# fbergama/wass

Hardware: AMD Instinct MI355X
Metric: stereo_pairs_per_sec (higher is better)
Workload: dtype u16

## Files before the change

### include/wass_gpu.h

```cpp
#ifndef WASS_GPU_H
#define WASS_GPU_H

#include <stddef.h>
#include <stdint.h>

#ifdef __cplusplus
extern "C" {
#endif

typedef enum {
    WASS_OK = 0,
    WASS_ERR_INVALID_ARG = -1,
    WASS_ERR_UNSUPPORTED = -2,
    WASS_ERR_NO_MEMORY = -3,
    WASS_ERR_DEVICE = -4,
    WASS_ERR_COST_OVERFLOW = -5,
    WASS_ERR_TOO_FEW_POINTS = -6
} wass_status;

typedef struct wass_ctx wass_ctx;

int wass_ctx_create(int device_id, wass_ctx** out);
int wass_device_count(int* n_devices);
void wass_ctx_destroy(wass_ctx* ctx);
// ... 123 lines not shown
typedef struct wass_debug_desc {
    int W0, H0;
    int roi_l[4], roi_r[4];
    const uint8_t* d_left_crop;
    const uint8_t* d_right_crop;
    const int16_t* d_disp16;
    const float* d_dispf;
    int num_disp, min_disp, disp_offset;
    double disparity_compensation;
    int quality;
} wass_debug_desc;
int wass_jpeg_encode_dev(wass_ctx* ctx, const uint8_t* d_pixels, int w, int h, int channels, size_t pitch_bytes, int quality,
                         uint8_t* h_dst, size_t capacity, size_t* nbytes);
int wass_debug_picture_size(const wass_debug_desc* desc, int k, int* width, int* height, int* channels);
int wass_debug_pictures_async(wass_ctx* ctx, const wass_mesh* mesh, const wass_debug_desc* desc, uint8_t* h_dst,
                              const size_t capacity[WASS_DEBUG_PICTURES], uint64_t* ticket);
int wass_debug_pictures_result(wass_ctx* ctx, uint64_t ticket, size_t nbytes[WASS_DEBUG_PICTURES]);

enum {
    WASS_CODE_NONE = 0,
    WASS_CODE_GREY = 1,
    WASS_CODE_OUTSIDE_IMAGE = 2,
    WASS_CODE_OUTSIDE_BBOX = 3,
    WASS_CODE_ANGLE = 4,
    WASS_CODE_TOO_CLOSE = 5,
    WASS_CODE_TOO_DISTANT = 6
};
int wass_mesh_reject_codes(wass_ctx* ctx, const wass_mesh* m, uint8_t* codes_out);
void wass_mesh_destroy(wass_mesh* m);
int wass_mesh_size(const wass_mesh* m, int* width, int* height);
int wass_mesh_download(wass_ctx* ctx, const wass_mesh* m, uint8_t* valid, double* p3d, uint8_t* gray);
int wass_mesh_upload(wass_ctx* ctx, int width, int height, const uint8_t* valid, const double* p3d,
                     const uint8_t* gray, wass_mesh** out);

int wass_mesh_zgap_percentile(wass_ctx* ctx, wass_mesh* m, double percentile, double* out, uint64_t* n_gaps);
int wass_mesh_keep_biggest_component(wass_ctx* ctx, wass_mesh* m, double zgap, uint64_t* size_out);
int wass_ransac_sample(int width, int height, int rounds, int32_t* uv_triplets);
int wass_ransac_sample_seeded(uint32_t seed, int width, int height, int rounds, int32_t* uv_triplets);
int wass_mesh_ransac_plane(wass_ctx* ctx, wass_mesh* m, const int32_t* uv_triplets, int rounds,
                           double thr, double plane_out[4], uint64_t* best_inliers, int* found);
int wass_mesh_crop_plane(wass_ctx* ctx, wass_mesh* m, const double plane[4], double thr, uint64_t* kept);
typedef struct {
    double xmin, xmax, ymin, ymax;
    double max_distance;
    int weight_by_distance;
    int central_third_only;
} wass_refine_params;
int wass_mesh_refine_plane(wass_ctx* ctx, wass_mesh* m, const wass_refine_params* rp,
                           double plane_out[4], uint64_t* n_inliers);
int wass_mesh_refinement_inliers(wass_ctx* ctx, wass_mesh* m, const wass_refine_params* rp, int every, double** xyz_out,
                                 uint64_t* n_out);
int wass_mesh_remove_outliers(wass_ctx* ctx, wass_mesh* m, double percentile, double* zgap_out, uint64_t* n_gaps,
                              uint64_t* size_out);
typedef struct {
    int      found;
    double   ransac_plane[4];
    uint64_t ransac_inliers;
    double   plane[4];
    uint64_t refine_inliers;
    uint64_t kept_after_ransac_crop, kept_final;
} wass_plane_result;
int wass_mesh_fit_plane(wass_ctx* ctx, wass_mesh* m, const int32_t* uv_triplets, int rounds, double ransac_thr,
                        const wass_refine_params* rp, double max_distance, wass_plane_result* out);
typedef struct {
    double   zgap;  uint64_t n_gaps, component_size;
    int      found, refine_ok;
    double   ransac_plane[4];  uint64_t ransac_inliers;
    double   plane[4];         uint64_t refine_inliers, kept_after_ransac_crop, kept_final;
    uint64_t n_points, xyzc_bytes;
    int      sgm_cost_overflow, sgm_timeout;
    uint64_t n_triangulated;
    uint64_t n_inliers_out;
    float stage_ms[5];
    int reserved;
    uint64_t inliers_text_bytes;
    uint32_t inliers_text_unsupported, reserved2;
} wass_frame_result;
int wass_mesh_finish_frame_async(wass_ctx* ctx, wass_mesh* m, double percentile, const int32_t* uv_triplets, int rounds,
                                 double ransac_thr, const wass_refine_params* rp, double max_distance, void* dst,
                                 size_t capacity);
int wass_mesh_finish_frame_async_ex(wass_ctx* ctx, wass_mesh* m, double percentile, const int32_t* uv_triplets, int rounds,
                                    double ransac_thr, const wass_refine_params* rp, double max_distance, void* dst,
                                    size_t capacity, double* inliers_dst, size_t inliers_capacity, int inliers_every,
                                    uint8_t* component_mask_dst);
int wass_mesh_finish_frame_async_ex2(wass_ctx* ctx, wass_mesh* m, double percentile, const int32_t* uv_triplets, int rounds,
                                     double ransac_thr, const wass_refine_params* rp, double max_distance, void* dst,
                                     size_t capacity, double* inliers_dst, size_t inliers_capacity, int inliers_every,
                                     uint8_t* component_mask_dst, char* inliers_text_dst, size_t inliers_text_capacity);
int wass_format_g6(double v, char* out);
int wass_ctx_frame_inliers(wass_ctx* ctx, double* dst, size_t capacity_points, uint64_t* n_out);
int wass_ctx_frame_result(wass_ctx* ctx, wass_frame_result* out);

void wass_RT_from_plane(const double plane[4], double R[9], double T[3], double Rinv[9], double Tinv[3]);
int wass_mesh_encode_xyzc(wass_ctx* ctx, wass_mesh* m, const double plane[4], void** bytes, size_t* nbytes);
int wass_mesh_encode_xyzc_to(wass_ctx* ctx, wass_mesh* m, const double plane[4], void* dst, size_t capacity,
                             size_t* nbytes);
int wass_mesh_encode_xyzc_async(wass_ctx* ctx, wass_mesh* m, const double plane[4], void* dst, size_t capacity,
                                size_t* nbytes);
void wass_free(void* p);

typedef struct {
    double R[9], T[3];
    double baseline;
    double xmin, xmax, ymin, ymax;
    int    width, height;
} wass_grid_setup;
// ... 210 lines not shown
```

### wass_amd/_lib.py

```python
from __future__ import annotations

import ctypes as C
import os

_HERE = os.path.dirname(os.path.abspath(__file__))
SO_PATH = os.environ.get("WASS_GPU_LIB") or os.path.join(_HERE, "libwassgpu.so")

WASS_OK = 0
WASS_ERR_COST_OVERFLOW = -5


class WassError(RuntimeError):
    def __init__(self, code: int, msg: str):
        super().__init__(f"libwassgpu error {code}: {msg}")
        self.code = code


class SgmParams(C.Structure):
    _fields_ = [(n, C.c_int) for n in (
        "min_disp", "num_disp", "win", "P1", "P2", "uniq_ratio", "disp12_max_diff", "prefilter_cap",
        "speckle_win", "speckle_range", "ndirs", "disp_offset")] + [("dense_scale", C.c_double)]


class SgmTimings(C.Structure):
# ... 69 lines not shown


def default_sgm_params(num_disp: int, ndirs: int = 5, min_disp: int = 1, win: int = 13, p1_mult: int = 2,
                       p2_mult: int = 64, disp_offset: int = 0) -> SgmParams:
    return SgmParams(min_disp, num_disp, win, p1_mult * win * win, p2_mult * win * win, 1, -1, 60, -70, 16,
                     ndirs, disp_offset, 1.0)


_vp, _i, _sz = C.c_void_p, C.c_int, C.c_size_t
SYMBOLS = {
    "wass_version": (C.c_char_p, []),
    "wass_ctx_create": (_i, [_i, C.POINTER(_vp)]),
    "wass_ctx_destroy": (None, [_vp]),
    "wass_last_error": (C.c_char_p, [_vp]),
    "wass_ctx_stream": (_vp, [_vp]),
    "wass_ctx_synchronize": (_i, [_vp]),
    "wass_ctx_set_debug": (_i, [_vp, _i]),
    "wass_ctx_set_tail_overlap": (_i, [_vp, _i]),
    "wass_sgm_disparity": (_i, [_vp, _vp, _vp, _i, _i, _sz, C.POINTER(SgmParams), _vp]),
    "wass_sgm_disparity_dev": (_i, [_vp, _vp, _vp, _i, _i, _sz, C.POINTER(SgmParams), _vp]),
    "wass_sgm_last_timings": (_i, [_vp, C.POINTER(SgmTimings)]),
    "wass_sgm_prev_timings": (_i, [_vp, C.POINTER(SgmTimings)]),
    "wass_sgm_call_count": (_i, [_vp, C.POINTER(C.c_uint64)]),
    "wass_sgm_call_timings": (_i, [_vp, C.c_uint64, C.POINTER(SgmTimings)]),
    "wass_sgm_debug_fetch": (_i, [_vp, _vp, _vp, _vp]),
    "wass_sgm_probe_vsum": (_i, [_vp, C.POINTER(C.c_float), C.POINTER(C.c_float)]),
    "wass_sgm_selftest": (_i, [_vp, _i, _i, _i, _i, C.POINTER(C.c_uint64)]),
    "wass_device_count": (_i, [C.POINTER(_i)]),
    "wass_ctx_set_kernel_events": (_i, [_vp, _i]),
    "wass_sgm_kernel_times": (_i, [_vp, C.c_char_p, C.c_size_t, C.POINTER(C.c_float), _i, C.POINTER(_i)]),
    "wass_disparity_postprocess": (_i, [_vp, _vp, _i, _i, C.POINTER(SgmParams), _i, _i, _i, _vp]),
    "wass_disparity_postprocess_dev": (_i, [_vp, _vp, _i, _i, C.POINTER(SgmParams), _i, _i, _i, _vp]),
    "wass_triangulate": (_i, [_vp, _vp, _i, _i, C.POINTER(_i), C.POINTER(_i), C.POINTER(Geom), _vp, _i, _i, _vp, _vp,
                              C.POINTER(TriParams), C.POINTER(_vp), C.POINTER(C.c_uint64)]),
    "wass_triangulate_dev": (_i, [_vp, _vp, _i, _i, C.POINTER(_i), C.POINTER(_i), C.POINTER(Geom), _vp, _i, _i, _vp, _vp,
                                  C.POINTER(TriParams), C.POINTER(_vp), C.POINTER(C.c_uint64)]),
    "wass_mesh_destroy": (None, [_vp]),
    "wass_mesh_size": (_i, [_vp, C.POINTER(_i), C.POINTER(_i)]),
    "wass_mesh_download": (_i, [_vp, _vp, _vp, _vp, _vp]),
    "wass_mesh_upload": (_i, [_vp, _i, _i, _vp, _vp, _vp, C.POINTER(_vp)]),
    "wass_mesh_zgap_percentile": (_i, [_vp, _vp, C.c_double, C.POINTER(C.c_double), C.POINTER(C.c_uint64)]),
    "wass_mesh_keep_biggest_component": (_i, [_vp, _vp, C.c_double, C.POINTER(C.c_uint64)]),
    "wass_ransac_sample": (_i, [_i, _i, _i, _vp]),
    "wass_ransac_sample_seeded": (_i, [C.c_uint32, _i, _i, _i, _vp]),
    "wass_mesh_ransac_plane": (_i, [_vp, _vp, _vp, _i, C.c_double, C.POINTER(C.c_double), C.POINTER(C.c_uint64),
                                    C.POINTER(_i)]),
    "wass_mesh_crop_plane": (_i, [_vp, _vp, C.POINTER(C.c_double), C.c_double, C.POINTER(C.c_uint64)]),
    "wass_large_gradient_mask": (_i, [_vp, _i, _i, _vp]),
    "wass_mesh_reject_codes": (_i, [_vp, _vp, _vp]),
    "wass_mesh_refine_plane": (_i, [_vp, _vp, C.POINTER(RefineParams), C.POINTER(C.c_double), C.POINTER(C.c_uint64)]),
    "wass_mesh_refinement_inliers": (_i, [_vp, _vp, C.POINTER(RefineParams), _i, C.POINTER(C.POINTER(C.c_double)), C.POINTER(C.c_uint64)]),
    "wass_mesh_remove_outliers": (_i, [_vp, _vp, C.c_double, C.POINTER(C.c_double), C.POINTER(C.c_uint64),
                                       C.POINTER(C.c_uint64)]),
    "wass_mesh_fit_plane": (_i, [_vp, _vp, _vp, _i, C.c_double, C.POINTER(RefineParams), C.c_double,
                                 C.POINTER(PlaneResult)]),
    "wass_RT_from_plane": (None, [C.POINTER(C.c_double)] * 5),
    "wass_mesh_encode_xyzc": (_i, [_vp, _vp, C.POINTER(C.c_double), C.POINTER(_vp), C.POINTER(_sz)]),
    "wass_mesh_encode_xyzc_to": (_i, [_vp, _vp, C.POINTER(C.c_double), _vp, _sz, C.POINTER(_sz)]),
    "wass_mesh_encode_xyzc_async": (_i, [_vp, _vp, C.POINTER(C.c_double), _vp, _sz, C.POINTER(_sz)]),
    "wass_mesh_finish_frame_async": (_i, [_vp, _vp, C.c_double, _vp, _i, C.c_double, C.POINTER(RefineParams), C.c_double, _vp, _sz]),
    "wass_mesh_finish_frame_async_ex": (_i, [_vp, _vp, C.c_double, _vp, _i, C.c_double, C.POINTER(RefineParams), C.c_double, _vp, _sz,
                                             _vp, _sz, _i, _vp]),
    "wass_mesh_finish_frame_async_ex2": (_i, [_vp, _vp, C.c_double, _vp, _i, C.c_double, C.POINTER(RefineParams), C.c_double, _vp, _sz,
                                              _vp, _sz, _i, _vp, _vp, _sz]),
    "wass_format_g6": (_i, [C.c_double, _vp]),
    "wass_ctx_frame_inliers": (_i, [_vp, _vp, _sz, C.POINTER(C.c_uint64)]),
    "wass_ctx_frame_result": (_i, [_vp, C.POINTER(FrameResult)]),
    "wass_device_alloc": (_i, [_vp, _sz, C.POINTER(_vp)]),
    "wass_device_free": (None, [_vp, _vp]),
    "wass_download": (_i, [_vp, _vp, _vp, _sz]),
    "wass_download_async": (_i, [_vp, _vp, _vp, _sz]),
    "wass_resize_cubic_u8_dev": (_i, [_vp, _vp, _i, _i, _sz, _vp, _i, _i]),
    "wass_jpeg_encode_dev": (_i, [_vp, _vp, _i, _i, _i, _sz, _i, _vp, _sz, C.POINTER(_sz)]),
    "wass_debug_pictures_async": (_i, [_vp, _vp, C.POINTER(DebugDesc), _vp, C.POINTER(_sz * 8), C.POINTER(C.c_uint64)]),
    "wass_debug_picture_size": (_i, [C.POINTER(DebugDesc), _i, C.POINTER(_i), C.POINTER(_i), C.POINTER(_i)]),
    "wass_debug_pictures_result": (_i, [_vp, C.c_uint64, C.POINTER(_sz * 8)]),
    "wass_pinned_alloc": (_i, [_vp, _sz, C.POINTER(_vp)]),
    "wass_pinned_free": (None, [_vp, _vp]),
    "wass_free": (None, [_vp]),
    "wass_mesh_grid_idw": (_i, [_vp, _vp, C.POINTER(GridSetup), _vp, _vp]),
    "wass_mesh_grid_idw_ex": (_i, [_vp, _vp, C.POINTER(GridSetup), _i, _vp, _vp]),
    "wass_dct_opts_default": (None, [C.POINTER(DctOpts)]),
    "wass_grid_dct": (_i, [_vp, _vp, _i, _i, C.POINTER(DctOpts), _vp, _vp, _vp, _vp, C.POINTER(DctInfo)]),
    "wass_grid_dct_dev": (_i, [_vp, _vp, _i, _i, C.POINTER(DctOpts), _vp, _vp, _vp, _vp, C.POINTER(DctInfo)]),
    "wass_mesh_grid_dct": (_i, [_vp, _vp, C.POINTER(GridSetup), _i, C.POINTER(DctOpts), _vp, _vp, _vp, _vp, _vp, C.POINTER(DctInfo)]),
    "wass_grid_dct_eval": (_i, [_vp, _vp, _i, _i, _i, C.c_double, _vp, _vp, C.POINTER(C.c_double), C.POINTER(C.c_double)]),
    "wass_grid_dct_batch": (_i, [_vp, _vp, _i, _i, _i, C.POINTER(DctOpts), _vp, _vp, _vp, _vp, C.POINTER(DctInfo), C.POINTER(_i)]),
    "wass_grid_dct_batch_dev": (_i, [_vp, _vp, _i, _i, _i, C.POINTER(DctOpts), _vp, _vp, _vp, _vp, C.POINTER(DctInfo), C.POINTER(_i)]),
    "wass_mesh_grid_cells_dev": (_i, [_vp, _vp, C.POINTER(GridSetup), _i, _vp]),
    "wass_grid_median_dev": (_i, [_vp, _vp, _vp, _i, _i, _i, _i, _vp]),
    "wass_grid_seq_create": (_i, [_vp, _i, _i, C.POINTER(_vp)]),
    "wass_grid_seq_push_dev": (_i, [_vp, _vp, _i, _vp]),
    "wass_grid_seq_finish": (_i, [_vp, _i, C.POINTER(GridSeqStats), _vp, _vp, _vp, _vp]),
    "wass_grid_seq_zero_mean_dev": (_i, [_vp, _vp, _i]),
    "wass_grid_seq_destroy": (None, [_vp]),
    "wass_spec3d_scratch_bytes": (_i, [_i, _i, _i, C.POINTER(_sz)]),
    "wass_spec3d_create": (_i, [_vp, _i, _i, _i, _vp, _vp, _vp, C.POINTER(_vp)]),
    "wass_spec3d_push": (_i, [_vp, _vp, _sz, _sz, C.c_double]),
    "wass_spec3d_push_dev": (_i, [_vp, _vp, _sz, _sz, C.c_double]),
    "wass_spec3d_finish": (_i, [_vp, C.c_double, _vp, C.POINTER(_i), C.POINTER(_i)]),
    "wass_spec3d_destroy": (None, [_vp]),
    "wass_spec1d_welch": (_i, [_vp, _vp, _i, _i, _i, C.c_double, C.c_double, _vp]),
    "wass_sosfiltfilt_scratch_bytes": (_i, [_i, _i, _i, _i, _i, _i, C.POINTER(_sz), C.POINTER(_i)]),
    "wass_sosfiltfilt": (_i, [_vp, _vp, _sz, _sz, _i, _i, _i, _vp, _i, _vp, _i, _i, _i, _vp, _sz, _sz]),
    "wass_sosfiltfilt_dev": (_i, [_vp, _vp, _sz, _sz, _i, _i, _i, _vp, _i, _vp, _i, _i, _i, _vp, _sz, _sz]),
    "wass_spatial_filter_scratch_bytes": (_i, [_i, _i, _i, C.POINTER(_sz)]),
# ... 91 lines not shown
```

### wass_amd/csrc/mesh.hip

```cpp
#include "common.h"
#include "fmt_g6.h"

#include <math.h>
#include <stdlib.h>
#include <mutex>
#include <new>
#include <vector>

namespace wass {

struct GeomDev {
    double Kl[9], Kr[9], R[9], T[3];
    int use_custom;
    double R1[9], R2[9], P1[12], P2[12], HLi[9], HRi[9];
    double comp_over_scale;
};

__device__ __forceinline__ void mulv(const double* M, const double* v, double* o)
{
    o[0] = M[0] * v[0] + M[1] * v[1] + M[2] * v[2];
    o[1] = M[3] * v[0] + M[4] * v[1] + M[5] * v[2];
    o[2] = M[6] * v[0] + M[7] * v[1] + M[8] * v[2];
}
__device__ __forceinline__ void tmulv(const double* M, const double* v, double* o)
// ... 274 lines not shown
            const unsigned int cm = (unsigned)((i % w) * h + (i / w));
            if (r == r0) { atomicAdd(&agg, (unsigned)len); atomicMin(&aggmin, cm); }
            else { atomicAdd(&size[r], (unsigned)len); atomicMin(&mincm[r], cm); }
        }
    }
    __syncthreads();
    if (threadIdx.x == 0 && agg) { atomicAdd(&size[r0], agg); atomicMin(&mincm[r0], aggmin); }
}
__global__ void __launch_bounds__(256) k_ccl_best(int n, const int* __restrict__ parent, const unsigned int* __restrict__ size,
                                                  const unsigned int* __restrict__ mincm, unsigned long long* __restrict__ best)
{
    const int i = blockIdx.x * 256 + threadIdx.x;
    unsigned long long key = 0;
    if (i < n && parent[i] == i) key = ((unsigned long long)size[i] << 32) | (unsigned long long)(0xFFFFFFFFu - mincm[i]);
    for (int o = 32; o > 0; o >>= 1) {
        const unsigned long long other = __shfl_down(key, o);
        key = other > key ? other : key;
    }
    if ((threadIdx.x & 63) == 0 && key) atomicMax(best, key);
}
__global__ void __launch_bounds__(256) k_ccl_keep(uint8_t* __restrict__ valid, int n, const int* __restrict__ parent,
                                                  const unsigned int* __restrict__ size, const unsigned int* __restrict__ mincm,
                                                  const unsigned long long* __restrict__ best)
{
    const int i = blockIdx.x * 256 + threadIdx.x;
    if (i >= n) return;
    const int r = parent[i];
    bool keep = false;
    if (r >= 0) {
        const unsigned long long key = ((unsigned long long)size[r] << 32) | (unsigned long long)(0xFFFFFFFFu - mincm[r]);
        keep = key == *best;
    }
    valid[i] = keep ? 1 : 0;
}

struct DevState {
    unsigned long long sel_k, sel_prefix, sel_total;
    int sel_hi_shift, sel_fail;
    double zgap;
    unsigned long long ccl_best;
    int ransac_found, pad0;
    unsigned long long ransac_best;
    double ransac_plane[4];
    double wsum, centroid[3], ninl;
    double plane[4];
    int refine_ok, pad1;
    double rtR[9], rtT[3], rtRinv[9], rtTinv[3];
    double mn[3], sc[3];
    unsigned int npts, have_plane;
    unsigned long long kept1, kept2;
    unsigned long long ntri;
    unsigned int ninl_sel, inl_text_bad;
    unsigned long long inl_text_bytes;
};

constexpr int GAP_HIST_COPIES = 4;
constexpr int GAP_BITS = 11, GAP_BINS = 1 << GAP_BITS, GAP_PASSES = 6;
__global__ void __launch_bounds__(256) k_gap_hist(const uint8_t* __restrict__ valid, const double* __restrict__ Z, int w, int h,
                                                  int shift, unsigned int mask, const DevState* __restrict__ ds,
                                                  unsigned int* __restrict__ hist)
{
    __shared__ unsigned int lh[GAP_BINS];
    for (int i = threadIdx.x; i < GAP_BINS; i += 256) lh[i] = 0;
    __syncthreads();
    const int hi_shift = ds->sel_hi_shift;
    const unsigned long long prefix = ds->sel_prefix;
    const int j = blockIdx.x * 256 + threadIdx.x;
    if (j >= 1 && j < w - 1)
        for (int i = 1 + blockIdx.y; i < h; i += gridDim.y) {
            const size_t c = (size_t)i * w + j, up = c - w;
            const uint8_t vc = valid[c], v0 = valid[up - 1], v1 = valid[up], v2 = valid[up + 1];
            const double z = Z[c], z0 = Z[up - 1], z1 = Z[up], z2 = Z[up + 1];
            if (!vc) continue;
            const double zn[3] = { z0, z1, z2 };
            const uint8_t vn[3] = { v0, v1, v2 };
#pragma unroll
            for (int k = 0; k < 3; ++k) {
                if (!vn[k]) continue;
                const unsigned long long key = (unsigned long long)__double_as_longlong(fabs(z - zn[k]));
                if (hi_shift < 64 && (key >> hi_shift) != prefix) continue;
                atomicAdd(&lh[(unsigned)(key >> shift) & mask], 1u);
            }
        }
    __syncthreads();
    unsigned int* mine = hist + (size_t)((blockIdx.x + blockIdx.y) % GAP_HIST_COPIES) * GAP_BINS;
    for (int i = threadIdx.x; i < GAP_BINS; i += 256)
        if (lh[i]) atomicAdd(&mine[i], lh[i]);
}
__global__ void __launch_bounds__(256) k_radix_pick(unsigned int* __restrict__ hist, int pass, int shift, int nbits,
                                                    double percentile, DevState* __restrict__ ds)
{
    __shared__ unsigned long long tot[256];
    const int nb = 1 << nbits, per = (nb + 255) / 256;
    for (int i = threadIdx.x; i < GAP_BINS; i += 256) {
        unsigned int t = hist[i];
        for (int cpy = 1; cpy < GAP_HIST_COPIES; ++cpy) t += hist[(size_t)cpy * GAP_BINS + i];
        hist[i] = t;
    }
    __syncthreads();
    unsigned long long s = 0;
    for (int b = threadIdx.x * per; b < min(nb, (threadIdx.x + 1) * per); ++b) s += hist[b];
    tot[threadIdx.x] = s;
    __syncthreads();
    if (threadIdx.x == 0) {
        unsigned long long k = ds->sel_k;
        if (pass == 0) {
            unsigned long long total = 0;
            for (int t = 0; t < 256; ++t) total += tot[t];
            ds->sel_total = total;
            k = (unsigned long long)floor(percentile / 100.0 * (double)total);
            if (total && k >= total) k = total - 1;
            ds->sel_prefix = 0;
            ds->sel_fail = total == 0;
        }
        if (!ds->sel_fail) {
            int t = 0;
            for (; t < 256; ++t) { if (k < tot[t]) break; k -= tot[t]; }
            int b = t * per;
            const int be = min(nb, (t + 1) * per);
            for (; b < be; ++b) { if (k < hist[b]) break; k -= hist[b]; }
            if (t >= 256 || b >= be) ds->sel_fail = 2;
            else {
                ds->sel_k = k;
                ds->sel_prefix = (ds->sel_prefix << nbits) | (unsigned long long)b;
                ds->sel_hi_shift = shift;
                if (shift == 0) ds->zgap = __longlong_as_double((long long)ds->sel_prefix);
            }
        }
        if (ds->sel_fail == 1) ds->zgap = __longlong_as_double(0x7FF8000000000000ll);
    }
    __syncthreads();
    for (int i = threadIdx.x; i < GAP_BINS * GAP_HIST_COPIES; i += 256) hist[i] = 0;
}

struct PlaneCand { double n[3]; double d; int ok; int pad; };

__global__ void k_ransac_planes(const uint8_t* __restrict__ valid, const double* __restrict__ X, const double* __restrict__ Y,
                                const double* __restrict__ Z, int w, const int32_t* __restrict__ uv, int rounds,
                                PlaneCand* __restrict__ cand, unsigned long long* __restrict__ counts,
                                unsigned long long* __restrict__ zero, int nzero)
{
    const int r = blockIdx.x * blockDim.x + threadIdx.x;
    for (int k = r; k < nzero; k += gridDim.x * blockDim.x) zero[k] = 0;
    if (r >= rounds) return;
    counts[r] = 0;
    const int32_t* c = uv + (size_t)r * 6;
    const size_t i1 = (size_t)c[1] * w + c[0], i2 = (size_t)c[3] * w + c[2], i3 = (size_t)c[5] * w + c[4];
    PlaneCand pc;
    pc.ok = valid[i1] && valid[i2] && valid[i3];
    pc.pad = 0;
    pc.n[0] = pc.n[1] = pc.n[2] = pc.d = 0.0;
    if (pc.ok) {
        const double a[3] = { X[i2] - X[i1], Y[i2] - Y[i1], Z[i2] - Z[i1] };
        const double b[3] = { X[i3] - X[i1], Y[i3] - Y[i1], Z[i3] - Z[i1] };
        double n[3] = { a[1] * b[2] - a[2] * b[1], a[2] * b[0] - a[0] * b[2], a[0] * b[1] - a[1] * b[0] };
        const double nn = sqrt(n[0] * n[0] + n[1] * n[1] + n[2] * n[2]);
        n[0] = n[0] / nn; n[1] = n[1] / nn; n[2] = n[2] / nn;
        if (n[2] < 0) { n[0] = n[0] * -1.0; n[1] = n[1] * -1.0; n[2] = n[2] * -1.0; }
        pc.n[0] = n[0]; pc.n[1] = n[1]; pc.n[2] = n[2];
        pc.d = -(n[0] * X[i1] + n[1] * Y[i1] + n[2] * Z[i1]);
    }
    cand[r] = pc;
}

typedef float f32x2 __attribute__((ext_vector_type(2)));

template <int PTS>
__global__ void __launch_bounds__(256) k_ransac_score(const uint8_t* __restrict__ valid, const double* __restrict__ X,
                                                      const double* __restrict__ Y, const double* __restrict__ Z, int w, int h,
                                                      const PlaneCand* __restrict__ cand, int rounds, double thr,
                                                      unsigned long long* __restrict__ counts)
{
    static_assert(PTS % 2 == 0, "points are processed in packed pairs");
    extern __shared__ __attribute__((aligned(16))) unsigned char smem[];
    double* pl = (double*)smem;
    unsigned int* lc = (unsigned int*)(pl + (size_t)rounds * 4);
    for (int r = threadIdx.x; r < rounds; r += 256) {
        pl[r * 4] = cand[r].n[0]; pl[r * 4 + 1] = cand[r].n[1]; pl[r * 4 + 2] = cand[r].n[2]; pl[r * 4 + 3] = cand[r].d;
        lc[r] = 0;
    }
    __syncthreads();
    const int lane = threadIdx.x & 63, wv = threadIdx.x >> 6;
    const int col = (blockIdx.x * 4 + wv) * 64 + lane, row0 = blockIdx.y * PTS;
    f32x2 px[PTS / 2], py[PTS / 2], pz[PTS / 2];
    unsigned long long vmask[PTS];
// ... 900 lines not shown
        ds->inl_text_bytes = have ? text_total[0] : 0ull;
        ds->inl_text_bad = have ? text_total[1] : 0u;
    }
    {
        unsigned long long k1 = 0, k2 = 0, k3 = 0;
        for (int i = threadIdx.x; i < NSLOT; i += 64) { k1 += kept[i]; k2 += kept[NSLOT + i]; k3 += tri ? tri[i] : 0ull; }
        for (int o = 32; o > 0; o >>= 1) { k1 += __shfl_down(k1, o); k2 += __shfl_down(k2, o); k3 += __shfl_down(k3, o); }
        if (threadIdx.x == 0) { ds->kept1 = k1; ds->kept2 = k2; ds->ntri = k3; ds->ninl_sel = inl_total && ds->ransac_found ? *inl_total : 0u; }
    }
    unsigned long long hl[6] = { ~0ull, ~0ull, ~0ull, 0, 0, 0 };
    for (int i = threadIdx.x; i < NSLOT; i += 64)
        for (int k = 0; k < 3; ++k) {
            if (lim[i * 6 + k] < hl[k]) hl[k] = lim[i * 6 + k];
            if (lim[i * 6 + 3 + k] > hl[3 + k]) hl[3 + k] = lim[i * 6 + 3 + k];
        }
    for (int o = 32; o > 0; o >>= 1)
        for (int k = 0; k < 3; ++k) {
            const unsigned long long a = __shfl_down(hl[k], o), b = __shfl_down(hl[3 + k], o);
            if (a < hl[k]) hl[k] = a;
            if (b > hl[3 + k]) hl[3 + k] = b;
        }
    if (threadIdx.x) return;
    const unsigned int npts = *total;
    double mx[3];
    for (int k = 0; k < 3; ++k) {
        ds->mn[k] = npts ? dunkey(hl[k]) : 1.7976931348623157e308;
        mx[k] = npts ? dunkey(hl[3 + k]) : -1.7976931348623157e308;
        ds->sc[k] = 65535.0 / (mx[k] - ds->mn[k]);
    }
    ds->npts = npts;
    unsigned int* w = (unsigned int*)img;
    w[0] = npts;
    auto put = [&](int word, double v) {
        const unsigned long long b = (unsigned long long)__double_as_longlong(v);
        w[word] = (unsigned int)b; w[word + 1] = (unsigned int)(b >> 32);
    };
    for (int k = 0; k < 3; ++k) put(1 + 2 * k, ds->sc[k]);
    for (int k = 0; k < 3; ++k) put(7 + 2 * k, ds->mn[k]);
    for (int k = 0; k < 9; ++k) put(13 + 2 * k, ds->rtRinv[k]);
    for (int k = 0; k < 3; ++k) put(31 + 2 * k, ds->rtTinv[k]);
}
__global__ void __launch_bounds__(256) k_xyzc_pack_dev(const uint8_t* __restrict__ valid, const double* __restrict__ X,
                                                       const double* __restrict__ Y, const double* __restrict__ Z, size_t n,
                                                       const DevState* __restrict__ ds, const unsigned int* __restrict__ blockoff,
                                                       uint16_t* __restrict__ out)
{
    RTDev rt;
    for (int i = 0; i < 9; ++i) rt.R[i] = ds->rtR[i];
    for (int i = 0; i < 3; ++i) rt.T[i] = ds->rtT[i];
    xyzc_pack_body(valid, X, Y, Z, n, rt, ds->mn[0], ds->mn[1], ds->mn[2], ds->sc[0], ds->sc[1], ds->sc[2], blockoff, out);
}

constexpr size_t DSTATE_HIST_OFF = (sizeof(DevState) + 255) & ~(size_t)255;
constexpr size_t DSTATE_STRIDE = (DSTATE_HIST_OFF + (size_t)GAP_HIST_COPIES * GAP_BINS * 4 + 255) & ~(size_t)255;
static int dstate(wass_ctx* c, DevState** ds)
{
    int rc = ensure(c, c->dstate, 2 * DSTATE_STRIDE);
    if (rc) return rc;
    *ds = (DevState*)((char*)c->dstate.p + (size_t)(c->ds_slot & 1) * DSTATE_STRIDE);
    return WASS_OK;
}

static int enqueue_ccl(wass_ctx* c, wass_mesh* m, DevState* ds)
{
    const size_t n = m->n();
    if (n > 0x7FFFFFFFull) return set_err(c, WASS_ERR_UNSUPPORTED, "mesh too large");
    int rc = ensure(c, c->scratch, n * 12);
    if (rc) return rc;
    int* parent = (int*)c->scratch.p;
    unsigned int* size = (unsigned int*)(parent + n);
    unsigned int* mincm = size + n;
    unsigned long long* best = &ds->ccl_best;
    const dim3 blk(256), g1(nblk(n));
    hipLaunchKernelGGL(k_ccl_init, g1, blk, 0, c->ts(), m->valid, m->z, m->w, (int)n, (const double*)&ds->zgap, parent, size, mincm, best);
    hipLaunchKernelGGL(k_ccl_merge, g1, blk, 0, c->ts(), m->valid, m->z, m->w, (int)n, (const double*)&ds->zgap, parent);
    hipLaunchKernelGGL(k_ccl_flatten, g1, blk, 0, c->ts(), (int)n, parent);
    hipLaunchKernelGGL(k_ccl_count, dim3((unsigned)((n + 1024 * CCL_COUNT_CHUNKS - 1) / (1024 * CCL_COUNT_CHUNKS))), dim3(1024), 0, c->ts(), (int)n, m->w, m->h,
                       (const int*)parent, size, mincm);
    hipLaunchKernelGGL(k_ccl_best, g1, blk, 0, c->ts(), (int)n, (const int*)parent, (const unsigned int*)size,
                       (const unsigned int*)mincm, best);
    hipLaunchKernelGGL(k_ccl_keep, g1, blk, 0, c->ts(), m->valid, (int)n, (const int*)parent, (const unsigned int*)size,
                       (const unsigned int*)mincm, (const unsigned long long*)best);
    WASS_HIP(c, hipGetLastError());
    return WASS_OK;
}

int wass_mesh_keep_biggest_component(wass_ctx* c, wass_mesh* m, double zgap, uint64_t* size_out)
{
    if (!c || !m) return set_err(c, WASS_ERR_INVALID_ARG, "null argument");
    WASS_HIP(c, hipSetDevice(c->device));
    DevState* ds = nullptr;
    int rc = dstate(c, &ds);
    if (rc) return rc;
    WASS_HIP(c, hipMemcpyAsync(&ds->zgap, &zgap, 8, hipMemcpyHostToDevice, c->ts()));
    WASS_HIP(c, hipStreamSynchronize(c->ts()));
    if ((rc = enqueue_ccl(c, m, ds))) return rc;
    if (size_out) {
        unsigned long long hb = 0;
        WASS_HIP(c, hipMemcpyAsync(&hb, &ds->ccl_best, 8, hipMemcpyDeviceToHost, c->ts()));
        WASS_HIP(c, hipStreamSynchronize(c->ts()));
        *size_out = hb >> 32;
    }
    return WASS_OK;
}

constexpr size_t STAGE_UV_OFF = 4096 + NSLOT * 6 * 8;
constexpr size_t STAGE_UV_BYTES = 1800 * 24;
constexpr size_t STAGE_BYTES = STAGE_UV_OFF + 2 * STAGE_UV_BYTES;
static int host_stage(wass_ctx* c, unsigned char** out)
{
    static_assert(sizeof(DevState) <= 4096, "DevState init image");
    if (!c->h_stage) {
        if (hipHostMalloc((void**)&c->h_stage, STAGE_BYTES, hipHostMallocDefault) != hipSuccess)
            return set_err(c, WASS_ERR_NO_MEMORY, "hipHostMalloc failed");
        unsigned char* p = (unsigned char*)c->h_stage;
        DevState init;
        memset(&init, 0, sizeof init);
        init.sel_hi_shift = 64;
        memcpy(p, &init, sizeof init);
        unsigned long long* lim = (unsigned long long*)(p + 4096);
        for (int i = 0; i < NSLOT; ++i) for (int k = 0; k < 6; ++k) lim[i * 6 + k] = k < 3 ? ~0ull : 0ull;
        if (hipEventCreateWithFlags(&c->ev_stage, hipEventDisableTiming) != hipSuccess || hipEventCreateWithFlags(&c->ev_stage2, hipEventDisableTiming) != hipSuccess)
            return set_err(c, WASS_ERR_DEVICE, "hipEventCreate failed");
    }
    *out = (unsigned char*)c->h_stage;
    return WASS_OK;
}

static int enqueue_remove_outliers(wass_ctx* c, wass_mesh* m, double percentile, DevState** dsp)
{
    DevState* ds = nullptr;
    int rc = dstate(c, &ds);
    if (rc) return rc;
    unsigned int* hist = (unsigned int*)((char*)ds + DSTATE_HIST_OFF);
    unsigned char* stage = nullptr;
    if ((rc = host_stage(c, &stage))) return rc;
    WASS_HIP(c, hipStreamWaitEvent(c->ts(), c->fslot[c->ds_slot & 1].ev_copy, 0));
    WASS_HIP(c, hipMemcpyAsync(ds, stage, sizeof(DevState), hipMemcpyHostToDevice, c->ts()));
    WASS_HIP(c, hipMemsetAsync(hist, 0, (size_t)GAP_HIST_COPIES * GAP_BINS * 4, c->ts()));
    for (int pass = 0; pass < GAP_PASSES; ++pass) {
        const int shift = pass < GAP_PASSES - 1 ? 64 - GAP_BITS * (pass + 1) : 0;
        const int nbits = pass < GAP_PASSES - 1 ? GAP_BITS : 64 - GAP_BITS * (GAP_PASSES - 1);
        hipLaunchKernelGGL(k_gap_hist, dim3((m->w + 255) / 256, 256), dim3(256), 0, c->ts(), m->valid, m->z, m->w, m->h, shift, (1u << nbits) - 1u,
                           (const DevState*)ds, hist);
        hipLaunchKernelGGL(k_radix_pick, dim3(1), dim3(256), 0, c->ts(), hist, pass, shift, nbits, percentile, ds);
    }
    if (c->ev_tail[2]) (void)hipEventRecord(c->ev_tail[2], c->ts());
    if ((rc = enqueue_ccl(c, m, ds))) return rc;
    if (c->ev_tail[3]) (void)hipEventRecord(c->ev_tail[3], c->ts());
    *dsp = ds;
    return WASS_OK;
}

int wass_mesh_remove_outliers(wass_ctx* c, wass_mesh* m, double percentile, double* zgap_out, uint64_t* n_gaps, uint64_t* size_out)
{
    if (!c || !m) return set_err(c, WASS_ERR_INVALID_ARG, "null argument");
    WASS_HIP(c, hipSetDevice(c->device));
    DevState* ds = nullptr;
    int rc = enqueue_remove_outliers(c, m, percentile, &ds);
    if (rc) return rc;
    DevState h;
    WASS_HIP(c, hipMemcpyAsync(&h, ds, sizeof h, hipMemcpyDeviceToHost, c->ts()));
    WASS_HIP(c, hipStreamSynchronize(c->ts()));
    if (h.sel_fail == 2) return set_err(c, WASS_ERR_DEVICE, "radix select lost its rank (internal error)");
    if (zgap_out) *zgap_out = h.zgap;
    if (n_gaps) *n_gaps = h.sel_total;
    if (size_out) *size_out = h.ccl_best >> 32;
    return WASS_OK;
}

}

template <typename Rand>
static int ransac_sample_with(Rand&& next, int width, int height, int rounds, int32_t* uv)
{
    if (width <= 0 || height <= 0 || rounds < 0 || !uv) return WASS_ERR_INVALID_ARG;
    const double mindist = height * 0.01;
    int r = 0;
    long guard = 0;
    while (r < rounds) {
        int p[6];
        for (int k = 0; k < 3; k++) { const int v = next() % height; const int u = next() % width; p[2 * k] = u; p[2 * k + 1] = v; }
        const double d12 = sqrt((double)(p[0] - p[2]) * (p[0] - p[2]) + (double)(p[1] - p[3]) * (p[1] - p[3]));
        const double d23 = sqrt((double)(p[2] - p[4]) * (p[2] - p[4]) + (double)(p[3] - p[5]) * (p[3] - p[5]));
        const double d13 = sqrt((double)(p[0] - p[4]) * (p[0] - p[4]) + (double)(p[1] - p[5]) * (p[1] - p[5]));
        if (d12 < mindist || d23 < mindist || d13 < mindist) {
            if (++guard > 100000000L) return WASS_ERR_INVALID_ARG;
            continue;
        }
        for (int k = 0; k < 6; k++) uv[(size_t)r * 6 + k] = p[k];
        r++;
    }
    return WASS_OK;
}

namespace {
struct GlibcRand {
    uint32_t r[34];
    int i = 0;
    explicit GlibcRand(uint32_t seed)
    {
        int32_t w[34];
        w[0] = seed == 0 ? 1 : (int32_t)seed;
        for (int k = 1; k < 31; ++k) {
            const long hi = w[k - 1] / 127773, lo = w[k - 1] % 127773;
            long word = 16807 * lo - 2836 * hi;
            if (word < 0) word += 2147483647;
            w[k] = (int32_t)word;
        }
        for (int k = 0; k < 31; ++k) r[k] = (uint32_t)w[k];
        for (int k = 31; k < 34; ++k) r[k] = r[k - 31];
        i = 0;
        for (int k = 0; k < 310; ++k) (void)next_word();
    }
    uint32_t next_word()
    {
        const uint32_t v = r[(i + 3) % 34] + r[(i + 31) % 34];
        r[i] = v;
        i = (i + 1) % 34;
        return v;
    }
// ... 552 lines not shown
```

### wass_amd/stereo.py

```python
from __future__ import annotations

import ctypes as C

import numpy as np

from . import _lib
from ._lib import (Geom, PlaneResult, RefineParams, SgmParams, SgmTimings, TriParams, WassError,
                   default_sgm_params)


def dense_input_size(w: int, h: int, dense_scale: float):
    ws, hs = C.c_int(), C.c_int()
    if _lib.load().wass_dense_input_size(w, h, C.c_double(dense_scale), C.byref(ws), C.byref(hs)) != 0:
        raise ValueError("bad DENSE_SCALE")
    return ws.value, hs.value


class Context:

    def __init__(self, device_id: int = 0):
        self._lib = _lib.load()
        h = C.c_void_p()
        rc = self._lib.wass_ctx_create(device_id, C.byref(h))
        if rc != 0:
# ... 528 lines not shown
        return valid, p3d, gray

    def grid_idw(self, plane=None, baseline: float = None, xmin: float = None, xmax: float = None, ymin: float = None, ymax: float = None,
                 width: int = None, height: int = None, cell: str = "mean", gs: "_lib.GridSetup" = None):
        if gs is None:
            R, T, _, _ = RT_from_plane(plane)
            gs = grid_setup(R, T, baseline, xmin, xmax, ymin, ymax, width, height)
        elif plane is not None:
            raise ValueError("grid_idw: give either gs or the plane, the baseline, the extent and the size")
        width, height = gs.width, gs.height
        grid = np.empty((height, width), np.float32); mask = np.empty((height, width), np.uint8)
        self.ctx._check(self.ctx._lib.wass_mesh_grid_idw_ex(self.ctx._h, self._h, C.byref(gs), {"mean": 0, "median": 1}[cell], grid.ctypes.data,
                                                            mask.ctypes.data))
        return grid, mask

    def grid_dct(self, plane, baseline: float, xmin: float, xmax: float, ymin: float, ymax: float, width: int, height: int,
                 cell: str = "mean", dct_options=None, x0=None, user_mask=None, seed: int = 0):
        gs = _lib.GridSetup()
        R, T, _, _ = RT_from_plane(plane)
        gs.R[:] = np.asarray(R, float).ravel().tolist(); gs.T[:] = np.asarray(T, float).ravel().tolist()
        gs.baseline, gs.xmin, gs.xmax, gs.ymin, gs.ymax, gs.width, gs.height = baseline, xmin, xmax, ymin, ymax, width, height
        o = dct_opts(dct_options, seed)
        x0c = None if x0 is None else np.ascontiguousarray(x0, np.float32).reshape(o.nfreqs, o.nfreqs)
        um = None if user_mask is None else np.ascontiguousarray(user_mask, np.uint8).reshape(height, width)
        grid = np.empty((height, width), np.float32); cells = np.empty((height, width), np.float32)
        coeffs = np.empty((max(o.nfreqs, 1), max(o.nfreqs, 1)), np.float32)
        info = _lib.DctInfo()
        self.ctx._check(self.ctx._lib.wass_mesh_grid_dct(self.ctx._h, self._h, C.byref(gs), {"mean": 0, "median": 1}[cell], C.byref(o),
                                                         None if x0c is None else x0c.ctypes.data, None if um is None else um.ctypes.data,
                                                         grid.ctypes.data, cells.ctypes.data, coeffs.ctypes.data, C.byref(info)))
        return grid, cells, coeffs, dct_info(info)

    def grid_cells_dev(self, gs: "_lib.GridSetup", d_cells, cell: str = "median"):
        if tuple(d_cells.shape) != (gs.height, gs.width) or not d_cells.is_contiguous():
            raise ValueError("d_cells: a contiguous float32 height x width tensor expected")
        self.ctx._check(self.ctx._lib.wass_mesh_grid_cells_dev(self.ctx._h, self._h, C.byref(gs), {"mean": 0, "median": 1}[cell],
                                                               d_cells.data_ptr()))

    def zgap_percentile(self, pct: float):
        out = C.c_double(); n = C.c_uint64()
        self.ctx._check(self.ctx._lib.wass_mesh_zgap_percentile(self.ctx._h, self._h, pct, C.byref(out), C.byref(n)))
        return out.value, int(n.value)

    def keep_biggest_component(self, zgap: float) -> int:
        n = C.c_uint64()
        self.ctx._check(self.ctx._lib.wass_mesh_keep_biggest_component(self.ctx._h, self._h, zgap, C.byref(n)))
        return int(n.value)

    def remove_outliers(self, pct: float):
        z = C.c_double(); n = C.c_uint64(); sz = C.c_uint64()
        self.ctx._check(self.ctx._lib.wass_mesh_remove_outliers(self.ctx._h, self._h, pct, C.byref(z), C.byref(n), C.byref(sz)))
        return z.value, int(n.value), int(sz.value)

    def fit_plane(self, uv, ransac_thr=1.0, max_distance=1.5, xmin=-9999., xmax=9999., ymin=-9999., ymax=9999.,
                  refine_max_distance=70.0, weight_by_distance=True, central_third_only=False) -> PlaneResult:
        uv = np.ascontiguousarray(uv, np.int32)
        rp = RefineParams(xmin, xmax, ymin, ymax, refine_max_distance, int(weight_by_distance), int(central_third_only))
        res = PlaneResult()
        self.ctx._check(self.ctx._lib.wass_mesh_fit_plane(self.ctx._h, self._h, uv.ctypes.data, len(uv), ransac_thr,
                                                          C.byref(rp), max_distance, C.byref(res)))
        return res

    def finish_frame_async(self, uv, dst_ptr: int, capacity: int, percentile=99.0, ransac_thr=1.0, max_distance=1.5,
                           xmin=-9999., xmax=9999., ymin=-9999., ymax=9999., refine_max_distance=70.0, weight_by_distance=True,
                           central_third_only=False, inliers_ptr: int = 0, inliers_capacity: int = 0, inliers_every: int = 10,
                           inliers_text_ptr: int = 0, inliers_text_capacity: int = 0, component_mask_ptr: int = 0) -> None:
        uv = np.ascontiguousarray(uv, np.int32)
        rp = RefineParams(xmin, xmax, ymin, ymax, refine_max_distance, int(weight_by_distance), int(central_third_only))
        if inliers_ptr or inliers_text_ptr or component_mask_ptr:
            self.ctx._check(self.ctx._lib.wass_mesh_finish_frame_async_ex2(self.ctx._h, self._h, percentile, uv.ctypes.data, len(uv), ransac_thr, C.byref(rp),
                                                                           max_distance, dst_ptr, capacity, inliers_ptr or None, inliers_capacity, inliers_every,
                                                                           component_mask_ptr or None,
                                                                           inliers_text_ptr or None, inliers_text_capacity))
            return
        self.ctx._check(self.ctx._lib.wass_mesh_finish_frame_async(self.ctx._h, self._h, percentile, uv.ctypes.data, len(uv),
                                                                   ransac_thr, C.byref(rp), max_distance, dst_ptr, capacity))

    def debug_pictures_async(self, desc: "_lib.DebugDesc", dst_ptr: int, capacities) -> int:
        caps = (C.c_size_t * 8)(*[int(c) for c in capacities])
        ticket = C.c_uint64()
        self.ctx._check(self.ctx._lib.wass_debug_pictures_async(self.ctx._h, self._h, C.byref(desc), dst_ptr, C.byref(caps), C.byref(ticket)))
        return int(ticket.value)

    def ransac_plane(self, uv, thr: float):
        uv = np.ascontiguousarray(uv, np.int32)
        plane = (C.c_double * 4)(); best = C.c_uint64(); found = C.c_int()
        self.ctx._check(self.ctx._lib.wass_mesh_ransac_plane(self.ctx._h, self._h, uv.ctypes.data, len(uv), thr, plane,
                                                             C.byref(best), C.byref(found)))
        return bool(found.value), np.array(plane[:]), int(best.value)

    def crop_plane(self, plane, thr: float) -> int:
        k = C.c_uint64()
        self.ctx._check(self.ctx._lib.wass_mesh_crop_plane(self.ctx._h, self._h, (C.c_double * 4)(*plane), thr, C.byref(k)))
        return int(k.value)

    def refine_plane(self, xmin=-9999., xmax=9999., ymin=-9999., ymax=9999., max_distance=70.0,
                     weight_by_distance=True, central_third_only=False):
        rp = RefineParams(xmin, xmax, ymin, ymax, max_distance, int(weight_by_distance), int(central_third_only))
        plane = (C.c_double * 4)(); n = C.c_uint64()
        self.ctx._check(self.ctx._lib.wass_mesh_refine_plane(self.ctx._h, self._h, C.byref(rp), plane, C.byref(n)))
        return np.array(plane[:]), int(n.value)

    def reject_codes(self):
        out = np.empty((self.height, self.width), np.uint8)
        self.ctx._check(self.ctx._lib.wass_mesh_reject_codes(self.ctx._h, self._h, out.ctypes.data))
        return out & 15, out >> 4
# ... 33 lines not shown
```

Baseline: 120.9.

## Fuse radix-pick into gap histogram and compact candidate gaps for later passes

Merges the separate percentile-pick kernel into the gap-histogram kernel through a last-block ticket, so each pass issues one launch instead of two. During an early pass, gap keys that match the current prefix are compacted into per-slot device lists. Later passes then build histograms from these short lists instead of re-scanning the full Z grid, and fall back to the full scan if a list overflows. The cost is extra device memory, atomics and ballot work in the listing pass, plus more complex cross-block synchronisation.

```diff
diff --git a/include/wass_gpu.h b/include/wass_gpu.h
--- a/include/wass_gpu.h
+++ b/include/wass_gpu.h
@@ -199,6 +199,8 @@
                                  uint64_t* n_out);
 int wass_mesh_remove_outliers(wass_ctx* ctx, wass_mesh* m, double percentile, double* zgap_out, uint64_t* n_gaps,
                               uint64_t* size_out);
+int wass_mesh_remove_outliers_ex(wass_ctx* ctx, wass_mesh* m, double percentile, unsigned int list_capacity, double* zgap_out,
+                                 uint64_t* n_gaps, uint64_t* size_out, int* list_used);
 typedef struct {
     int      found;
     double   ransac_plane[4];
diff --git a/wass_amd/_lib.py b/wass_amd/_lib.py
--- a/wass_amd/_lib.py
+++ b/wass_amd/_lib.py
@@ -145,6 +145,8 @@
     "wass_mesh_refinement_inliers": (_i, [_vp, _vp, C.POINTER(RefineParams), _i, C.POINTER(C.POINTER(C.c_double)), C.POINTER(C.c_uint64)]),
     "wass_mesh_remove_outliers": (_i, [_vp, _vp, C.c_double, C.POINTER(C.c_double), C.POINTER(C.c_uint64),
                                        C.POINTER(C.c_uint64)]),
+    "wass_mesh_remove_outliers_ex": (_i, [_vp, _vp, C.c_double, C.c_uint, C.POINTER(C.c_double), C.POINTER(C.c_uint64),
+                                          C.POINTER(C.c_uint64), C.POINTER(C.c_int)]),
     "wass_mesh_fit_plane": (_i, [_vp, _vp, _vp, _i, C.c_double, C.POINTER(RefineParams), C.c_double,
                                  C.POINTER(PlaneResult)]),
     "wass_RT_from_plane": (None, [C.POINTER(C.c_double)] * 5),
diff --git a/wass_amd/csrc/mesh.hip b/wass_amd/csrc/mesh.hip
--- a/wass_amd/csrc/mesh.hip
+++ b/wass_amd/csrc/mesh.hip
@@ -350,54 +350,39 @@
     unsigned long long ntri;
     unsigned int ninl_sel, inl_text_bad;
     unsigned long long inl_text_bytes;
+    unsigned int sel_ticket, list_over, list_done, pad2;
 };
 
 constexpr int GAP_HIST_COPIES = 4;
 constexpr int GAP_BITS = 11, GAP_BINS = 1 << GAP_BITS, GAP_PASSES = 6;
-__global__ void __launch_bounds__(256) k_gap_hist(const uint8_t* __restrict__ valid, const double* __restrict__ Z, int w, int h,
-                                                  int shift, unsigned int mask, const DevState* __restrict__ ds,
-                                                  unsigned int* __restrict__ hist)
-{
-    __shared__ unsigned int lh[GAP_BINS];
-    for (int i = threadIdx.x; i < GAP_BINS; i += 256) lh[i] = 0;
+constexpr int GAP_LIST_PASS = 2;
+constexpr unsigned int GAP_LIST_SEG_CAP = 1024;
+
+__device__ __forceinline__ void gap_pass_end(unsigned int* lh, unsigned long long* tot, unsigned int* last, unsigned int* __restrict__ hist,
+                                             unsigned int copy, unsigned int nwg, int pass, int shift, int nbits, double percentile,
+                                             bool closes_list, DevState* ds)
+{
     __syncthreads();
-    const int hi_shift = ds->sel_hi_shift;
-    const unsigned long long prefix = ds->sel_prefix;
-    const int j = blockIdx.x * 256 + threadIdx.x;
-    if (j >= 1 && j < w - 1)
-        for (int i = 1 + blockIdx.y; i < h; i += gridDim.y) {
-            const size_t c = (size_t)i * w + j, up = c - w;
-            const uint8_t vc = valid[c], v0 = valid[up - 1], v1 = valid[up], v2 = valid[up + 1];
-            const double z = Z[c], z0 = Z[up - 1], z1 = Z[up], z2 = Z[up + 1];
-            if (!vc) continue;
-            const double zn[3] = { z0, z1, z2 };
-            const uint8_t vn[3] = { v0, v1, v2 };
-#pragma unroll
-            for (int k = 0; k < 3; ++k) {
-                if (!vn[k]) continue;
-                const unsigned long long key = (unsigned long long)__double_as_longlong(fabs(z - zn[k]));
-                if (hi_shift < 64 && (key >> hi_shift) != prefix) continue;
-                atomicAdd(&lh[(unsigned)(key >> shift) & mask], 1u);
-            }
-        }
+    if (threadIdx.x < 64) {
+        unsigned int* mine = hist + (size_t)copy * GAP_BINS;
+        for (int i = threadIdx.x; i < GAP_BINS; i += 64)
+            if (lh[i]) atomicAdd(&mine[i], lh[i]);
+        __threadfence();
+        if (threadIdx.x == 0) *last = atomicAdd(&ds->sel_ticket, 1u) == nwg - 1u;
+    }
     __syncthreads();
-    unsigned int* mine = hist + (size_t)((blockIdx.x + blockIdx.y) % GAP_HIST_COPIES) * GAP_BINS;
-    for (int i = threadIdx.x; i < GAP_BINS; i += 256)
-        if (lh[i]) atomicAdd(&mine[i], lh[i]);
-}
-__global__ void __launch_bounds__(256) k_radix_pick(unsigned int* __restrict__ hist, int pass, int shift, int nbits,
-                                                    double percentile, DevState* __restrict__ ds)
-{
-    __shared__ unsigned long long tot[256];
+    if (!*last) return;
+    __threadfence();
+    for (int i = threadIdx.x; i < GAP_BINS; i += 256) {
+        unsigned int t = 0;
+        for (int cpy = 0; cpy < GAP_HIST_COPIES; ++cpy)
+            t += __hip_atomic_load(&hist[(size_t)cpy * GAP_BINS + i], __ATOMIC_RELAXED, __HIP_MEMORY_SCOPE_AGENT);
+        lh[i] = t;
+    }
+    __syncthreads();
     const int nb = 1 << nbits, per = (nb + 255) / 256;
-    for (int i = threadIdx.x; i < GAP_BINS; i += 256) {
-        unsigned int t = hist[i];
-        for (int cpy = 1; cpy < GAP_HIST_COPIES; ++cpy) t += hist[(size_t)cpy * GAP_BINS + i];
-        hist[i] = t;
-    }
-    __syncthreads();
     unsigned long long s = 0;
-    for (int b = threadIdx.x * per; b < min(nb, (threadIdx.x + 1) * per); ++b) s += hist[b];
+    for (int b = threadIdx.x * per; b < min(nb, ((int)threadIdx.x + 1) * per); ++b) s += lh[b];
     tot[threadIdx.x] = s;
     __syncthreads();
     if (threadIdx.x == 0) {
@@ -416,7 +401,7 @@
             for (; t < 256; ++t) { if (k < tot[t]) break; k -= tot[t]; }
             int b = t * per;
             const int be = min(nb, (t + 1) * per);
-            for (; b < be; ++b) { if (k < hist[b]) break; k -= hist[b]; }
+            for (; b < be; ++b) { if (k < lh[b]) break; k -= lh[b]; }
             if (t >= 256 || b >= be) ds->sel_fail = 2;
             else {
                 ds->sel_k = k;
@@ -426,9 +411,85 @@
             }
         }
         if (ds->sel_fail == 1) ds->zgap = __longlong_as_double(0x7FF8000000000000ll);
-    }
+        if (closes_list) ds->list_done = __hip_atomic_load(&ds->list_over, __ATOMIC_RELAXED, __HIP_MEMORY_SCOPE_AGENT) ? 0u : 1u;
+        ds->sel_ticket = 0;
+    }
+    for (int i = threadIdx.x; i < GAP_BINS * GAP_HIST_COPIES; i += 256) hist[i] = 0;
+}
+
+__global__ void __launch_bounds__(256) k_gap_hist(const uint8_t* __restrict__ valid, const double* __restrict__ Z, int w, int h,
+                                                  int pass, int shift, int nbits, double percentile, DevState* ds,
+                                                  unsigned int* __restrict__ hist, unsigned long long* __restrict__ list,
+                                                  unsigned int* __restrict__ lcnt, unsigned int seg_cap)
+{
+    __shared__ unsigned int lh[GAP_BINS];
+    __shared__ unsigned long long tot[256];
+    __shared__ unsigned int last;
+    if (ds->list_done) return;
+    for (int i = threadIdx.x; i < GAP_BINS; i += 256) lh[i] = 0;
     __syncthreads();
-    for (int i = threadIdx.x; i < GAP_BINS * GAP_HIST_COPIES; i += 256) hist[i] = 0;
+    const int hi_shift = ds->sel_hi_shift;
+    const unsigned long long prefix = ds->sel_prefix;
+    const unsigned int mask = (1u << nbits) - 1u;
+    const int j = blockIdx.x * 256 + threadIdx.x;
+    const int lane = threadIdx.x & 63;
+    const size_t seg = (size_t)slot_of_block();
+    bool over = false, set_over = false;
+    if (j >= 1 && j < w - 1)
+        for (int i = 1 + blockIdx.y; i < h; i += gridDim.y) {
+            const size_t c = (size_t)i * w + j, up = c - w;
+            const uint8_t vc = valid[c], v0 = valid[up - 1], v1 = valid[up], v2 = valid[up + 1];
+            const double z = Z[c], z0 = Z[up - 1], z1 = Z[up], z2 = Z[up + 1];
+            const double zn[3] = { z0, z1, z2 };
+            const uint8_t vn[3] = { v0, v1, v2 };
+#pragma unroll
+            for (int k = 0; k < 3; ++k) {
+                const unsigned long long key = (unsigned long long)__double_as_longlong(fabs(z - zn[k]));
+                const bool match = vc && vn[k] && (hi_shift >= 64 || (key >> hi_shift) == prefix);
+                if (match) atomicAdd(&lh[(unsigned)(key >> shift) & mask], 1u);
+                if (!list) continue;
+                const unsigned long long m = __ballot(match);
+                if (!m || over) continue;
+                over = __hip_atomic_load(&ds->list_over, __ATOMIC_RELAXED, __HIP_MEMORY_SCOPE_AGENT) != 0;
+                if (over) continue;
+                const int leader = __ffsll((long long)m) - 1;
+                const unsigned int cnt = (unsigned)__popcll(m);
+                unsigned int base = 0;
+                if (lane == leader) base = atomicAdd(&lcnt[seg], cnt);
+                base = __shfl(base, leader);
+                if (base + cnt > seg_cap) {
+                    if (lane == leader) __hip_atomic_store(&ds->list_over, 1u, __ATOMIC_RELAXED, __HIP_MEMORY_SCOPE_AGENT);
+                    over = set_over = true;
+                } else if (match)
+                    list[seg * GAP_LIST_SEG_CAP + base + (unsigned)__popcll(m & ((1ull << lane) - 1ull))] = key;
+            }
+        }
+    if (set_over) __threadfence();
+    gap_pass_end(lh, tot, &last, hist, (blockIdx.x + blockIdx.y) % GAP_HIST_COPIES, gridDim.x * gridDim.y, pass, shift, nbits, percentile,
+                 list != nullptr, ds);
+}
+__global__ void __launch_bounds__(256) k_gap_list_hist(const unsigned long long* __restrict__ list, const unsigned int* __restrict__ lcnt,
+                                                       int pass, int shift, int nbits, double percentile, DevState* ds,
+                                                       unsigned int* __restrict__ hist)
+{
+    __shared__ unsigned int lh[GAP_BINS];
+    __shared__ unsigned long long tot[256];
+    __shared__ unsigned int last;
+    if (!ds->list_done) return;
+    for (int i = threadIdx.x; i < GAP_BINS; i += 256) lh[i] = 0;
+    __syncthreads();
+    const int hi_shift = ds->sel_hi_shift;
+    const unsigned long long prefix = ds->sel_prefix;
+    const unsigned int mask = (1u << nbits) - 1u;
+    for (unsigned int seg = blockIdx.x; seg < (unsigned)NSLOT; seg += gridDim.x) {
+        const unsigned int cnt = min(lcnt[seg], GAP_LIST_SEG_CAP);
+        for (unsigned int i = threadIdx.x; i < cnt; i += 256) {
+            const unsigned long long key = list[(size_t)seg * GAP_LIST_SEG_CAP + i];
+            if ((key >> hi_shift) != prefix) continue;
+            atomicAdd(&lh[(unsigned)(key >> shift) & mask], 1u);
+        }
+    }
+    gap_pass_end(lh, tot, &last, hist, blockIdx.x % GAP_HIST_COPIES, gridDim.x, pass, shift, nbits, percentile, false, ds);
 }
 
 struct PlaneCand { double n[3]; double d; int ok; int pad; };
@@ -1435,7 +1496,9 @@
 }
 
 constexpr size_t DSTATE_HIST_OFF = (sizeof(DevState) + 255) & ~(size_t)255;
-constexpr size_t DSTATE_STRIDE = (DSTATE_HIST_OFF + (size_t)GAP_HIST_COPIES * GAP_BINS * 4 + 255) & ~(size_t)255;
+constexpr size_t DSTATE_LCNT_OFF = DSTATE_HIST_OFF + (size_t)GAP_HIST_COPIES * GAP_BINS * 4;
+constexpr size_t DSTATE_LIST_OFF = DSTATE_LCNT_OFF + (size_t)NSLOT * 4;
+constexpr size_t DSTATE_STRIDE = (DSTATE_LIST_OFF + (size_t)NSLOT * GAP_LIST_SEG_CAP * 8 + 255) & ~(size_t)255;
 static int dstate(wass_ctx* c, DevState** ds)
 {
     int rc = ensure(c, c->dstate, 2 * DSTATE_STRIDE);
@@ -1510,23 +1573,29 @@
     return WASS_OK;
 }
 
-static int enqueue_remove_outliers(wass_ctx* c, wass_mesh* m, double percentile, DevState** dsp)
+static int enqueue_remove_outliers(wass_ctx* c, wass_mesh* m, double percentile, DevState** dsp, unsigned int list_capacity = 0)
 {
     DevState* ds = nullptr;
     int rc = dstate(c, &ds);
     if (rc) return rc;
     unsigned int* hist = (unsigned int*)((char*)ds + DSTATE_HIST_OFF);
+    unsigned int* lcnt = (unsigned int*)((char*)ds + DSTATE_LCNT_OFF);
+    unsigned long long* list = (unsigned long long*)((char*)ds + DSTATE_LIST_OFF);
+    const unsigned int seg_cap = list_capacity ? std::min(list_capacity / NSLOT, GAP_LIST_SEG_CAP) : GAP_LIST_SEG_CAP;
     unsigned char* stage = nullptr;
     if ((rc = host_stage(c, &stage))) return rc;
     WASS_HIP(c, hipStreamWaitEvent(c->ts(), c->fslot[c->ds_slot & 1].ev_copy, 0));
     WASS_HIP(c, hipMemcpyAsync(ds, stage, sizeof(DevState), hipMemcpyHostToDevice, c->ts()));
-    WASS_HIP(c, hipMemsetAsync(hist, 0, (size_t)GAP_HIST_COPIES * GAP_BINS * 4, c->ts()));
+    WASS_HIP(c, hipMemsetAsync(hist, 0, DSTATE_LIST_OFF - DSTATE_HIST_OFF, c->ts()));
+    const dim3 walk((unsigned)std::max(1, (m->w + 255) / 256), 256);
     for (int pass = 0; pass < GAP_PASSES; ++pass) {
         const int shift = pass < GAP_PASSES - 1 ? 64 - GAP_BITS * (pass + 1) : 0;
         const int nbits = pass < GAP_PASSES - 1 ? GAP_BITS : 64 - GAP_BITS * (GAP_PASSES - 1);
-        hipLaunchKernelGGL(k_gap_hist, dim3((m->w + 255) / 256, 256), dim3(256), 0, c->ts(), m->valid, m->z, m->w, m->h, shift, (1u << nbits) - 1u,
-                           (const DevState*)ds, hist);
-        hipLaunchKernelGGL(k_radix_pick, dim3(1), dim3(256), 0, c->ts(), hist, pass, shift, nbits, percentile, ds);
+        if (pass > GAP_LIST_PASS)
+            hipLaunchKernelGGL(k_gap_list_hist, dim3(NSLOT), dim3(256), 0, c->ts(), (const unsigned long long*)list, (const unsigned int*)lcnt, pass,
+                               shift, nbits, percentile, ds, hist);
+        hipLaunchKernelGGL(k_gap_hist, walk, dim3(256), 0, c->ts(), m->valid, m->z, m->w, m->h, pass, shift, nbits, percentile, ds, hist,
+                           pass == GAP_LIST_PASS ? list : (unsigned long long*)nullptr, lcnt, seg_cap);
     }
     if (c->ev_tail[2]) (void)hipEventRecord(c->ev_tail[2], c->ts());
     if ((rc = enqueue_ccl(c, m, ds))) return rc;
@@ -1535,12 +1604,13 @@
     return WASS_OK;
 }
 
-int wass_mesh_remove_outliers(wass_ctx* c, wass_mesh* m, double percentile, double* zgap_out, uint64_t* n_gaps, uint64_t* size_out)
+int wass_mesh_remove_outliers_ex(wass_ctx* c, wass_mesh* m, double percentile, unsigned int list_capacity, double* zgap_out, uint64_t* n_gaps,
+                                 uint64_t* size_out, int* list_used)
 {
     if (!c || !m) return set_err(c, WASS_ERR_INVALID_ARG, "null argument");
     WASS_HIP(c, hipSetDevice(c->device));
     DevState* ds = nullptr;
-    int rc = enqueue_remove_outliers(c, m, percentile, &ds);
+    int rc = enqueue_remove_outliers(c, m, percentile, &ds, list_capacity);
     if (rc) return rc;
     DevState h;
     WASS_HIP(c, hipMemcpyAsync(&h, ds, sizeof h, hipMemcpyDeviceToHost, c->ts()));
@@ -1549,7 +1619,13 @@
     if (zgap_out) *zgap_out = h.zgap;
     if (n_gaps) *n_gaps = h.sel_total;
     if (size_out) *size_out = h.ccl_best >> 32;
-    return WASS_OK;
+    if (list_used) *list_used = (int)h.list_done;
+    return WASS_OK;
+}
+
+int wass_mesh_remove_outliers(wass_ctx* c, wass_mesh* m, double percentile, double* zgap_out, uint64_t* n_gaps, uint64_t* size_out)
+{
+    return wass_mesh_remove_outliers_ex(c, m, percentile, 0, zgap_out, n_gaps, size_out, nullptr);
 }
 
 }
diff --git a/wass_amd/stereo.py b/wass_amd/stereo.py
--- a/wass_amd/stereo.py
+++ b/wass_amd/stereo.py
@@ -604,6 +604,12 @@
         self.ctx._check(self.ctx._lib.wass_mesh_remove_outliers(self.ctx._h, self._h, pct, C.byref(z), C.byref(n), C.byref(sz)))
         return z.value, int(n.value), int(sz.value)
 
+    def remove_outliers_ex(self, pct: float, list_capacity: int = 0):
+        z = C.c_double(); n = C.c_uint64(); sz = C.c_uint64(); used = C.c_int()
+        self.ctx._check(self.ctx._lib.wass_mesh_remove_outliers_ex(self.ctx._h, self._h, pct, int(list_capacity), C.byref(z), C.byref(n),
+                                                                   C.byref(sz), C.byref(used)))
+        return z.value, int(n.value), int(sz.value), bool(used.value)
+
     def fit_plane(self, uv, ransac_thr=1.0, max_distance=1.5, xmin=-9999., xmax=9999., ymin=-9999., ymax=9999.,
                   refine_max_distance=70.0, weight_by_distance=True, central_third_only=False) -> PlaneResult:
         uv = np.ascontiguousarray(uv, np.int32)
```

Result: slower. 118.0 (-2.4%).
